# joekurina/Agilex-NTT

Measured on AMD Instinct MI355X. Metric: batched n=4096 forward NTTs/sec at 1/2/4/8 MI355X; %HBM roofline, higher is better.
Workload: dtype u64; 1 GPU; n=4096, 4-prime RNS (60-bit), batch=4096 polynomials per GPU, forward negacyclic NTT in place (BASELINE.json configs[2]); n=4096, primes=4, batch_per_gpu=4096, slabs_rotated=4, clock_ramp_steps_before_warmup=2240, parallelism=batch-sharded x1, no collective

## Files before the change

### agilex-ntt_amd/csrc/modarith.hpp

```cpp
#pragma once
#include <hip/hip_runtime.h>
#include <cstdint>

#include "q60c_class.hpp"

namespace agx {

typedef ulonglong2 twpair;

__device__ __forceinline__ uint64_t mul_shoup_lazy(uint64_t y, uint64_t w, uint64_t wp, uint64_t q) {
    const uint64_t c = __umul64hi(y, wp);
    return w * y - c * q;
}

__device__ __forceinline__ uint64_t csub(uint64_t v, uint64_t m) { return v >= m ? v - m : v; }

__device__ __forceinline__ uint64_t reduce_4q(uint64_t v, uint64_t q, uint64_t q2) {
    return csub(csub(v, q2), q);
}

__device__ __forceinline__ void ct_butterfly(uint64_t& x, uint64_t& y, uint64_t w, uint64_t wp,
                                             uint64_t q, uint64_t q2) {
    const uint64_t tx = csub(x, q2);
    const uint64_t qv = mul_shoup_lazy(y, w, wp, q);
    x = tx + qv;
    y = tx + q2 - qv;
}

__device__ __forceinline__ void gs_butterfly(uint64_t& x, uint64_t& y, uint64_t w, uint64_t wp,
                                             uint64_t q, uint64_t q2) {
    const uint64_t s = csub(x + y, q2);
    const uint64_t d = x + q2 - y;
    x = s;
    y = mul_shoup_lazy(d, w, wp, q);
}

struct barrett128 {
    uint64_t q;
    uint64_t mu_hi, mu_lo;
};

__device__ __forceinline__ uint64_t mul_mod_barrett(uint64_t a, uint64_t b, const barrett128& k) {
    const uint64_t lo = a * b, hi = __umul64hi(a, b);
    const uint64_t est = hi * k.mu_hi + __umul64hi(hi, k.mu_lo) + __umul64hi(lo, k.mu_hi);
    uint64_t r = lo - est * k.q;
    r = csub(r, k.q << 1);
    return csub(r, k.q);
}


__device__ __forceinline__ uint64_t reduce_u64(uint64_t v, const barrett128& k) {
    return csub(v - __umul64hi(v, k.mu_hi) * k.q, k.q);
}

__device__ __forceinline__ uint64_t rescale_lift(uint64_t t, uint64_t h, uint64_t hq, uint64_t q_last, const barrett128& k) {
    const uint64_t a = reduce_u64(csub(t + h, q_last), k);
    return a - hq + (a < hq ? k.q : 0);
}
template <bool LAZY>
__device__ __forceinline__ uint64_t rescale_finish(uint64_t x, uint64_t z, uint64_t w, uint64_t wp, uint64_t q) {
    const uint64_t d = x + (LAZY ? q << 2 : q) - z;
    return csub(mul_shoup_lazy(d, w, wp, q), q);
}

__device__ __forceinline__ uint64_t basis_scale(uint64_t x, uint64_t w, uint64_t wp, uint64_t qi) {
    return csub(mul_shoup_lazy(x, w, wp, qi), qi);
}
__device__ __forceinline__ uint64_t basis_accumulate(uint64_t acc, uint64_t y, uint64_t c, uint64_t cp, uint64_t q, uint64_t q2) {
    return csub(acc + mul_shoup_lazy(y, c, cp, q), q2);
}


__device__ __forceinline__ uint64_t mad64(uint32_t a, uint32_t b, uint64_t c) { return (uint64_t)a * b + c; }
__device__ __forceinline__ uint64_t mul64(uint32_t a, uint32_t b) { return (uint64_t)a * b; }

template <int TAG>
__device__ __forceinline__ uint32_t opaque_one() {
    uint32_t one;
    if constexpr (TAG == 0) asm("s_mov_b32 %0, 1" : "=s"(one));
    else asm("s_movk_i32 %0, 0x1" : "=s"(one));
    return one;
}
__device__ __forceinline__ uint64_t add64_32(uint64_t c, uint32_t a, uint32_t one) { return (uint64_t)a * one + c; }

__device__ __forceinline__ uint64_t opaque_sgpr64(uint64_t v) {
    asm("" : "+s"(v));
    return v;
}

__device__ __forceinline__ uint64_t keep64(uint64_t v) {
    asm("" : "+v"(v));
    return v;
}

struct bf_consts {
    uint64_t q;
    uint64_t nq;
    uint64_t m;
    uint64_t nm;
    uint32_t one_a, one_b;
    float est_inv;
    uint32_t c, c8;
    uint32_t c2, p29;
    uint64_t mfold;
};

__device__ __forceinline__ uint64_t csub_sign(uint64_t x, const bf_consts& k) {
    const uint64_t d = x + k.nm;
    const uint32_t neg = (uint32_t)((int32_t)(uint32_t)(d >> 32) >> 31);
    typedef uint32_t u32x2 __attribute__((ext_vector_type(2)));
    u32x2 add;
    add.x = neg & (uint32_t)k.m;
    add.y = neg & (uint32_t)(k.m >> 32);
    return d + __builtin_bit_cast(uint64_t, add);
}

template <int VAR = 0>
__device__ __forceinline__ uint64_t fold_product(uint64_t tx, uint64_t y, uint64_t w, uint64_t c, const bf_consts& k) {
    const uint32_t y0 = (uint32_t)y, y1 = (uint32_t)(y >> 32), w0 = (uint32_t)w, w1 = (uint32_t)(w >> 32);
    const uint32_t c0 = (uint32_t)c, c1 = (uint32_t)(c >> 32), nq0 = (uint32_t)k.nq, nq1 = (uint32_t)(k.nq >> 32);
    uint64_t acc = mad64(w0, y0, tx);
    acc = mad64(nq0, c0, acc);
    if constexpr (VAR == 1) {
        const uint32_t z32 = w0 * y1 + w1 * y0 + nq1 * c0 + nq0 * c1;
        typedef uint32_t u32x2v __attribute__((ext_vector_type(2)));
        u32x2v av = __builtin_bit_cast(u32x2v, acc);
        av.y += z32;
        return __builtin_bit_cast(uint64_t, av);
    }
    uint64_t z = mul64(w0, y1);
    z = mad64(w1, y0, z);
    z = mad64(nq1, c0, z);
    z = keep64(mad64(nq0, c1, z));
    typedef uint32_t u32x2 __attribute__((ext_vector_type(2)));
    u32x2 a = __builtin_bit_cast(u32x2, acc);
    a.y += (uint32_t)z;
    return __builtin_bit_cast(uint64_t, a);
}

__device__ __forceinline__ void ct_butterfly_exact(uint64_t& x, uint64_t& y, uint64_t w, uint64_t wp, const bf_consts& k) {
    const uint32_t y0 = (uint32_t)y, y1 = (uint32_t)(y >> 32), p0 = (uint32_t)wp, p1 = (uint32_t)(wp >> 32);
    const uint64_t tx = csub(x, k.m);
    const uint32_t t = __umulhi(y0, p0);
    const uint64_t m1 = add64_32(mul64(p1, y0), t, k.one_a);
    const uint64_t m2 = add64_32(mul64(p0, y1), (uint32_t)m1, k.one_b);
    uint64_t c = add64_32(mul64(p1, y1), (uint32_t)(m1 >> 32), k.one_a);
    c = add64_32(c, (uint32_t)(m2 >> 32), k.one_b);
    const uint64_t xn = fold_product(tx, y, w, c, k);
    y = (tx << 1) + k.m - xn;
    x = xn;
}

__device__ __forceinline__ uint64_t csub_select(uint64_t x, const bf_consts& k) {
    const uint64_t d = x + k.nm;
    return (int64_t)d < 0 ? x : d;
}

template <bool SEL = false>
__device__ __forceinline__ void ct_butterfly_fast(uint64_t& x, uint64_t& y, uint64_t w, uint64_t wp, const bf_consts& k) {
    const uint32_t y0 = (uint32_t)y, y1 = (uint32_t)(y >> 32), p0 = (uint32_t)wp, p1 = (uint32_t)(wp >> 32);
    const uint64_t tx = SEL ? csub_select(x, k) : csub_sign(x, k);
    uint64_t c = mad64(p1, y1, (uint64_t)__umulhi(y0, p1));
    c = add64_32(c, __umulhi(y1, p0), k.one_b);
    const uint64_t xn = fold_product(tx, y, w, c, k);
    y = (tx << 1) + k.m - xn;
    x = xn;
}

__device__ __forceinline__ uint64_t csub_sign_c(uint64_t x, uint64_t m, uint64_t nm) {
    const uint64_t d = x + nm;
    const uint32_t neg = (uint32_t)((int32_t)(uint32_t)(d >> 32) >> 31);
    typedef uint32_t u32x2 __attribute__((ext_vector_type(2)));
    u32x2 add;
    add.x = neg & (uint32_t)m;
    add.y = neg & (uint32_t)(m >> 32);
    return d + __builtin_bit_cast(uint64_t, add);
}

struct final_consts {
    uint64_t q2, nq2, q1, nq1;
    uint64_t q8, nq8;
};

template <bool FAST, bool SEL = false>
__device__ __forceinline__ uint64_t reduce_final(uint64_t v, const bf_consts& k, const final_consts& f, bool lazy_out = false) {
    if constexpr (FAST && SEL) {
        const uint64_t d4 = v + k.nm;
        v = (int64_t)d4 < 0 ? v : d4;
        if (lazy_out) return v;
        const uint64_t d2 = v + f.nq2;
        v = (int64_t)d2 < 0 ? v : d2;
        const uint64_t d1 = v + f.nq1;
        return (int64_t)d1 < 0 ? v : d1;
    } else if constexpr (FAST) {
        v = csub_sign(v, k);
        if (lazy_out) return v;
        v = csub_sign_c(v, f.q2, f.nq2);
        return csub_sign_c(v, f.q1, f.nq1);
    } else {
        if (lazy_out) return v;
        v = csub(v, k.q << 1);
        return csub(v, k.q);
    }
}

struct lazy16_schedule {
    static constexpr int bound_in(int s) {
        int b = 4;
        for (int i = 0; i < s; ++i) b = next(b);
        return b;
    }
    static constexpr bool subtracts(int s) { return bound_in(s) + 4 > 16; }
    static constexpr int next(int b) { return (b + 4 > 16 ? (b - 8 > 8 ? b - 8 : 8) : b) + 4; }
};

struct lazy16_tailfree {
    static constexpr bool subtracts(int s, int total) { return s >= 2 && (((s ^ total) & 1) == 0); }
    static constexpr int bound_in(int s, int total) {
        int b = 4;
        for (int i = 0; i < s; ++i) {
            if (subtracts(i, total)) b = b - 8 > 8 ? b - 8 : 8;
            b += 4;
        }
        return b;
    }
    static constexpr bool valid(int total) {
        for (int s = 0; s < total; ++s) {
            const int in = bound_in(s, total);
            if (in > 16) return false;
            if (!subtracts(s, total) && in + 4 > 16) return false;
        }
        return total >= 3 && !subtracts(total - 1, total);
    }
};

__device__ __forceinline__ uint64_t csub_select_c(uint64_t x, uint64_t nm) {
    const uint64_t d = x + nm;
    return (int64_t)d < 0 ? x : d;
}

template <bool SEL, bool DO_CSUB, bool LAST = false, int VAR = 0>
__device__ __forceinline__ void ct_butterfly_lazy16(uint64_t& x, uint64_t& y, uint64_t w, uint64_t wp, const bf_consts& k,
                                                    const final_consts& f) {
    const uint32_t y0 = (uint32_t)y, y1 = (uint32_t)(y >> 32), p0 = (uint32_t)wp, p1 = (uint32_t)(wp >> 32);
    uint64_t tx = x;
    if constexpr (DO_CSUB || LAST) {
        if constexpr (SEL) tx = csub_select_c(tx, f.nq8);
        else tx = csub_sign_c(tx, f.q8, f.nq8);
    }
    if constexpr (LAST) {
        if constexpr (SEL) tx = csub_select_c(tx, k.nm);
        else tx = csub_sign(tx, k);
    }
    uint64_t c = mad64(p1, y1, (uint64_t)__umulhi(y0, p1));
    c = add64_32(c, __umulhi(y1, p0), k.one_b);
    const uint64_t xn = fold_product<VAR>(tx, y, w, c, k);
    y = (tx << 1) + k.m - xn;
    x = xn;
}

template <bool SEL>
__device__ __forceinline__ uint64_t reduce_final_lazy16(uint64_t v, const bf_consts& k, const final_consts& f, bool lazy_out) {
    if constexpr (SEL) {
        v = csub_select_c(v, k.nm);
        if (lazy_out) return v;
        v = csub_select_c(v, f.nq2);
        return csub_select_c(v, f.nq1);
    } else {
        v = csub_sign(v, k);
        if (lazy_out) return v;
        v = csub_sign_c(v, f.q2, f.nq2);
        return csub_sign_c(v, f.q1, f.nq1);
    }
}

template <bool SEL, int USE_EST = -1>
__device__ __forceinline__ uint64_t reduce_final_est(uint64_t v, const bf_consts& k, const final_consts& f, bool lazy_out) {
    static_assert(SEL, "select-based conditional subtract only");
    if (USE_EST == 1 || (USE_EST == -1 && k.est_inv != 0.0f)) {
        const uint32_t kq = (uint32_t)((float)(uint32_t)(v >> 32) * k.est_inv);
        typedef uint32_t u32x2 __attribute__((ext_vector_type(2)));
        u32x2 r = __builtin_bit_cast(u32x2, mad64(kq, (uint32_t)k.nq, v));
        r.y += kq * (uint32_t)(k.nq >> 32);
        const uint64_t r64 = __builtin_bit_cast(uint64_t, r);
        return lazy_out ? r64 : csub_select_c(r64, f.nq1);
    }
    v = csub_select_c(v, f.nq8);
    v = csub_select_c(v, k.nm);
    if (lazy_out) return v;
    v = csub_select_c(v, f.nq2);
    return csub_select_c(v, f.nq1);
}

struct q60c_tailfree {
    struct bound {
        int b, e;
    };
    static constexpr bound bound_in(int s, int total) {
        bound v{4, 0};
        for (int i = 0; i < s; ++i) {
            if (lazy16_tailfree::subtracts(i, total)) {
                v.b = v.b - 8 > 8 ? v.b - 8 : 8;
                v.e = v.e > 1 ? v.e : 1;
            }
            v.b += 4;
        }
        return v;
    }
    static constexpr bool valid(int total) {
        for (int s = 0; s <= total; ++s) {
            const bound v = bound_in(s, total);
            if (v.b > 16 || v.e > 1) return false;
        }
        return lazy16_tailfree::valid(total);
    }
};

__device__ __forceinline__ uint64_t csub_8q_q60c(uint64_t x, const bf_consts& k) {
    typedef uint32_t u32x2 __attribute__((ext_vector_type(2)));
    u32x2 v = __builtin_bit_cast(u32x2, x);
    uint32_t s = v.y >> 31;
    asm("" : "+v"(s));
    v.y &= 0x7fffffffu;
    return mad64(s, k.c8, __builtin_bit_cast(uint64_t, v));
}

template <bool DO_CSUB>
__device__ __forceinline__ void ct_butterfly_q60c(uint64_t& x, uint64_t& y, uint64_t w, uint64_t wp, const bf_consts& k) {
    const uint32_t y0 = (uint32_t)y, y1 = (uint32_t)(y >> 32), p0 = (uint32_t)wp, p1 = (uint32_t)(wp >> 32);
    const uint64_t tx = DO_CSUB ? csub_8q_q60c(x, k) : x;
    uint64_t c = mad64(p1, y1, (uint64_t)__umulhi(y0, p1));
    c = add64_32(c, __umulhi(y1, p0), k.one_b);
    const uint64_t xn = fold_product(tx, y, w, c, k);
    y = (tx << 1) + k.m - xn;
    x = xn;
}

template <bool PIN = false>
__device__ __forceinline__ uint64_t reduce_top4_q60c(uint64_t x, const bf_consts& k) {
    typedef uint32_t u32x2 __attribute__((ext_vector_type(2)));
    u32x2 r = __builtin_bit_cast(u32x2, x);
    uint32_t kq = r.y >> 28;
    if constexpr (PIN) asm("" : "+v"(kq));
    r.y &= 0x0fffffffu;
    return mad64(kq, k.c, __builtin_bit_cast(uint64_t, r));
}
__device__ __forceinline__ uint64_t reduce_final_q60c(uint64_t v, const bf_consts& k, const final_consts& f, bool lazy_out) {
    const uint64_t t = reduce_top4_q60c(v, k);
    return lazy_out ? t : csub_select_c(t, f.nq1);
}

struct q60c_fold_bounds {
    typedef unsigned __int128 u128;
    static constexpr u128 two64 = (u128)1 << 64, w32 = 0xffffffffull;
    static constexpr u128 c_max = (1ull << 28) - 1, q_min = (1ull << 60) - (uint64_t)c_max, q_max = (1ull << 60) - 1;
    static constexpr u128 wh_max = (uint64_t)q_max >> 29, wl_max = (1ull << 29) - 1;
    static constexpr u128 hi_max = 2 * w32 * wh_max;
    static constexpr u128 lo_max = 2 * w32 * wl_max;
    static constexpr u128 Q_max = lo_max + w32 * ((u128)1 << 29) + w32 * 2 * c_max;
    static constexpr u128 tx_max = ((u128)1 << 63) + 8 * c_max - 1, tx_max_c1 = ((u128)1 << 63) + 8 - 1;
    static_assert(wh_max < ((u128)1 << 31), "the high half of a twiddle fits 31 bits");
    static_assert(hi_max < two64, "hi fits 64 bits");
    static_assert(tx_max + Q_max < two64, "x' = tx + Q does not wrap (every partial sum of the chain is below this one)");
    static_assert(Q_max <= 8 * q_min, "y' = tx + 8q - Q is not negative");
    static_assert(tx_max + 8 * q_min < two64 && tx_max_c1 + 8 * q_max < two64, "y' <= tx + 8q = 2^64 - 1 for every c");
};

__device__ __forceinline__ uint32_t opaque_two29() {
    uint32_t v;
    asm("s_mov_b32 %0, 0x20000000" : "=s"(v));
    return v;
}

struct q60c_skip_schedule {
    static constexpr bool reduces(int s) { return (s & 1) == 0; }
    static constexpr bool valid(int total) {
        for (int s = 1; s < total; ++s)
            if (!reduces(s) && !reduces(s - 1)) return false;
        return total >= 1 && reduces(0);
    }
};
struct q60c_skip_bounds {
    typedef unsigned __int128 u128;
    using F = q60c_fold_bounds;
    static constexpr u128 two64 = F::two64, w32 = F::w32;
    static constexpr u128 c_max = kQ60cSkipMaxC, q_min = (1ull << 60) - (uint64_t)c_max;
    static constexpr u128 Q_max = F::lo_max + w32 * ((u128)1 << 29) + w32 * 2 * c_max;
    static constexpr u128 r_max = ((u128)1 << 60) - 1 + 15 * c_max;
    static constexpr u128 out1_max = r_max + 7 * q_min;
    static_assert(c_max < ((u128)1 << 28), "a subclass of the moduli of q60c_fold_bounds: hi and the halves of a twiddle are bounded there");
    static_assert(15 * c_max < ((u128)1 << 32), "the fold's product fits a word");
    static_assert(Q_max <= 7 * q_min, "y' = tx + 7q - Q is not negative, on either kind of stage");
    static_assert(out1_max == ((u128)1 << 63) + 8 * c_max - 1, "8q + 16c - 1");
    static_assert(r_max + Q_max < two64, "reducing stage: x' does not wrap (every partial sum of the chain is below this one)");
    static_assert(out1_max + Q_max < two64, "the stage behind it: x' does not wrap (every partial sum of the chain is below this one)");
    static_assert(out1_max + 7 * q_min < two64, "... and y' <= tx + 7q = 15 2^60 + c - 1 (grows with c) stays below 2^64");
};

template <int FORM>
__device__ __forceinline__ void ct_butterfly_q60c_fold(uint64_t& x, uint64_t& y, uint64_t w, uint64_t wC, const bf_consts& k) {
    static_assert(FORM >= 0 && FORM <= 3, "no such form");
    const uint32_t y0 = (uint32_t)y, y1 = (uint32_t)(y >> 32);
    const uint32_t wl = (uint32_t)w, wh = (uint32_t)(w >> 32), wCl = (uint32_t)wC, wCh = (uint32_t)(wC >> 32);
    const uint64_t tx = FORM == 1 ? csub_8q_q60c(x, k) : FORM == 2 ? reduce_top4_q60c<true>(x, k) : x;
    const uint64_t hi = mad64(y1, wCh, mul64(y0, wh));
    uint64_t xn = keep64(mad64(y0, wl, tx));
    xn = mad64(y1, wCl, xn);
    xn = mad64((uint32_t)hi, k.p29, xn);
    xn = mad64((uint32_t)(hi >> 32), k.c2, xn);
    y = (tx << 1) + k.mfold - xn;
    x = xn;
}

template <bool FAST>
__device__ __forceinline__ uint64_t mul_shoup_form(uint64_t d, uint64_t w, uint64_t wp, const bf_consts& k) {
    const uint32_t d0 = (uint32_t)d, d1 = (uint32_t)(d >> 32), p0 = (uint32_t)wp, p1 = (uint32_t)(wp >> 32);
    uint64_t c;
    if constexpr (FAST) {
        c = mad64(p1, d1, (uint64_t)__umulhi(d0, p1));
        c = add64_32(c, __umulhi(d1, p0), k.one_b);
    } else {
        const uint32_t t = __umulhi(d0, p0);
        const uint64_t m1 = add64_32(mul64(p1, d0), t, k.one_a);
        const uint64_t m2 = add64_32(mul64(p0, d1), (uint32_t)m1, k.one_b);
        c = add64_32(mul64(p1, d1), (uint32_t)(m1 >> 32), k.one_a);
        c = add64_32(c, (uint32_t)(m2 >> 32), k.one_b);
    }
    return fold_product(0, d, w, c, k);
}

template <bool FAST, bool SEL = false>
__device__ __forceinline__ void gs_butterfly_form(uint64_t& x, uint64_t& y, uint64_t w, uint64_t wp, const bf_consts& k) {
    const uint64_t s = x + y;
    const uint64_t d = x + k.m - y;
    if constexpr (FAST) x = SEL ? csub_select(s, k) : csub_sign(s, k);
    else x = csub(s, k.m);
    y = mul_shoup_form<FAST>(d, w, wp, k);
}

template <bool FAST>
__device__ __forceinline__ void gs_last_form(uint64_t& x, uint64_t& y, uint64_t ninv, uint64_t ninv_p,
                                             uint64_t w1n, uint64_t w1n_p, const bf_consts& k) {
    const uint64_t s = x + y;
    const uint64_t d = x + k.m - y;
    x = mul_shoup_form<FAST>(s, ninv, ninv_p, k);
    y = mul_shoup_form<FAST>(d, w1n, w1n_p, k);
}

template <bool SEL>
__device__ __forceinline__ uint64_t csub_8q(uint64_t v, const final_consts& f) {
    return SEL ? csub_select_c(v, f.nq8) : csub_sign_c(v, f.q8, f.nq8);
}
constexpr int gs_bound(int B0, int s, int r) {
    if (s == 0) return B0;
    if ((r >> (s - 1)) & 1) return 4;
    const int b = gs_bound(B0, s - 1, r);
    return 2 * (b == 16 ? 8 : b);
}
template <int B, bool SEL>
__device__ __forceinline__ void gs_butterfly_lazy16(uint64_t& x, uint64_t& y, uint64_t w, uint64_t wp, const bf_consts& k, const final_consts& f) {
    static_assert(B == 4 || B == 8 || B == 16, "bounds are 4q, 8q or 16q");
    if constexpr (B == 16) {
        x = csub_8q<SEL>(x, f);
        y = csub_8q<SEL>(y, f);
    }
    const uint64_t s = x + y;
    const uint64_t d = x + (B == 4 ? k.m : f.q8) - y;
    y = mul_shoup_form<true>(d, w, wp, k);
    x = s;
}
template <int B, bool SEL>
__device__ __forceinline__ void gs_last_lazy16(uint64_t& x, uint64_t& y, uint64_t ninv, uint64_t ninv_p, uint64_t w1n, uint64_t w1n_p,
                                               const bf_consts& k, const final_consts& f) {
    if constexpr (B == 16) {
        x = csub_8q<SEL>(x, f);
        y = csub_8q<SEL>(y, f);
    }
    const uint64_t s = x + y;
    const uint64_t d = x + (B == 4 ? k.m : f.q8) - y;
    x = mul_shoup_form<true>(s, ninv, ninv_p, k);
    y = mul_shoup_form<true>(d, w1n, w1n_p, k);
}

template <bool FAST, bool SEL = false>
__device__ __forceinline__ uint64_t reduce_final_inv(uint64_t v, const bf_consts& k, const final_consts& f) {
    if constexpr (FAST && SEL) {
        v = csub_select_c(v, f.nq2);
        return csub_select_c(v, f.nq1);
    } else if constexpr (FAST) {
        v = csub_sign_c(v, f.q2, f.nq2);
        return csub_sign_c(v, f.q1, f.nq1);
    } else {
        return csub(v, k.q);
    }
}

}
```

### agilex-ntt_amd/csrc/rb_frame.hpp

```cpp
#pragma once
#include "rb_registry.hpp"
#include "modarith.hpp"

#include <algorithm>
#include <cstdlib>
#include <type_traits>
#include <utility>

#ifndef AGX_POLYMUL_MAXW
#define AGX_POLYMUL_MAXW 5
#endif
#ifndef AGX_TU
#error "define AGX_TU (a per-translation-unit namespace name) before including rb_frame.hpp / rb_kernels.hpp"
#endif

namespace agx {
namespace AGX_TU {



template <int B, int E, typename F>
__device__ __host__ __forceinline__ void static_for(F&& f) {
    if constexpr (B < E) {
        f(std::integral_constant<int, B>{});
        static_for<B + 1, E>(std::forward<F>(f));
    }
}

extern __shared__ __attribute__((aligned(16))) unsigned char agx_dyn_lds[];

template <int L, int R>
struct rb_geom {
    static constexpr int C = 1 << R;
    static constexpr int T = 1 << (L - R);
    static constexpr int NP = (L + R - 1) / R;
    static constexpr int rlo(int p) { return (L - R * (p + 1)) > 0 ? (L - R * (p + 1)) : 0; }
    static constexpr int hi(int p) { return L - 1 - R * p; }
    static constexpr int H(int p) { return 1 << (L - R - rlo(p)); }
    static constexpr int table_off(int p) { return p == 0 ? 0 : table_off(p - 1) + C * H(p - 1); }
    static constexpr int table_pairs = table_off(NP);
};

template <int L, int R>
struct rb2_geom : rb_geom<L, R> {
    using G = rb_geom<L, R>;
    static constexpr uint32_t elem(int p, uint32_t tid, uint32_t r) {
        const int rlo = G::rlo(p);
        return (tid & ((1u << rlo) - 1u)) | (r << rlo) | ((tid >> rlo) << (rlo + R));
    }
    static constexpr uint32_t owner(int p, uint32_t e) {
        const int rlo = G::rlo(p);
        return (e & ((1u << rlo) - 1u)) | ((e >> (rlo + R)) << rlo);
    }
    static constexpr bool exchange_is_wave_local(int p) {
        for (uint32_t tid = 0; tid < (uint32_t)G::T; ++tid)
            for (uint32_t r = 0; r < (uint32_t)G::C; ++r)
                if ((owner(p + 1, elem(p, tid, r)) >> 6) != (tid >> 6)) return false;
        return true;
    }
    static constexpr bool uniform_pass(int p) { return G::rlo(p) >= 6 || G::H(p) == 1; }
    static constexpr bool last_pass_wave_contiguous() { return G::rlo(G::NP - 1) == 0 && G::T >= 64; }
};

__device__ __forceinline__ twpair load_uniform(const twpair* p) {
    typedef const uint64_t __attribute__((address_space(4))) * const_ptr;
    const_ptr c = (const_ptr)(uintptr_t)p;
    twpair r;
    r.x = c[0];
    r.y = c[1];
    return r;
}

__device__ __forceinline__ void wave_lds_sync() {
    __builtin_amdgcn_fence(__ATOMIC_RELEASE, "wavefront");
    __builtin_amdgcn_wave_barrier();
    __builtin_amdgcn_fence(__ATOMIC_ACQUIRE, "wavefront");
}

struct bf_regs {
    int r0, r1, o;
};
template <int rb>
constexpr bf_regs bf_pair(int b) {
    const int r0 = ((b >> rb) << (rb + 1)) | (b & ((1 << rb) - 1));
    return {r0, r0 | (1 << rb), b >> rb};
}

struct no_op {
    __device__ __forceinline__ void operator()() const {}
};
template <int C, class WR, class RD, class SYNC, class MID = no_op>
__device__ __forceinline__ void split_words_out(const uint64_t (&x)[C], uint32_t* w, uint32_t (&lo)[C], WR&& wr, RD&& rd, SYNC&& sync, MID&& mid = MID{}) {
    static_for<0, C>([&](auto r) { w[wr(r)] = (uint32_t)x[r]; });
    mid();
    sync();
    static_for<0, C>([&](auto r) { lo[r] = w[rd(r)]; });
    sync();
    static_for<0, C>([&](auto r) { w[wr(r)] = (uint32_t)(x[r] >> 32); });
    sync();
}

constexpr int kOptPad = 1;
constexpr int kOptSelect = 2;
constexpr int kOptLazy16 = 16;
constexpr int kOptTwAhead = 32;
constexpr int kOptTrace = 64;
constexpr int kOptPrio = 128;
constexpr int kOptPrioBarrier = 512;
constexpr int kOptScalarBase = 1024;
constexpr int kOptLazyInv = 2048;
constexpr int kOptTwAheadInv = 4096;
constexpr int kOptNtLoad = 131072, kOptNtStore = 262144;
constexpr int kOptEstReduce = 524288;
constexpr int kOptSplitWord = 1048576;
constexpr int kOptStreamTw = 1 << 25;
constexpr int kOptPinBf = 1 << 26;
constexpr int kOptQ60c = 1 << 27;
constexpr int kOptQ60cFold = 1 << 28;
constexpr int kOptQ60cSkip = 1 << 21;
constexpr int kOptStreamCh1 = 1 << 29;

#ifdef AGX_DIAG
__device__ uint64_t* g_trace_buf = nullptr;
__device__ uint64_t g_trace_waves = 0;
#endif

template <int L, int R, bool FAST, int OPT = 0>
struct rb2_frame {
    using G = rb2_geom<L, R>;
    static constexpr int C = G::C, T = G::T, NP = G::NP;
    static constexpr bool FAST_ARITH = FAST, SEL = (OPT & kOptSelect) != 0, LAZY16 = FAST && (OPT & kOptLazy16) != 0;
    static_assert((OPT & kOptPad) != 0, "every kernel uses the padded image");
    static constexpr bool TWA = (OPT & kOptTwAhead) != 0 && R >= 3;
    static constexpr bool TRACE = (OPT & kOptTrace) != 0;
    static constexpr bool PRIO = (OPT & kOptPrio) != 0;
    static constexpr bool PRIO_BARRIER = PRIO && (OPT & kOptPrioBarrier) != 0, SCALAR_BASE = (OPT & kOptScalarBase) != 0;
    static constexpr bool LAZY_INV = LAZY16 && (OPT & kOptLazyInv) != 0;
    static constexpr bool NT_LOAD = (OPT & kOptNtLoad) != 0, NT_STORE = (OPT & kOptNtStore) != 0;
    static constexpr bool TWA_INV = (OPT & kOptTwAheadInv) != 0 && R == 3;
    static constexpr bool EST = LAZY16 && SEL && (OPT & kOptEstReduce) != 0;
    static constexpr bool Q60C = EST && (OPT & kOptQ60c) != 0;
    static constexpr bool Q60C_FOLD = Q60C && (OPT & kOptQ60cFold) != 0;
    static_assert((OPT & kOptQ60cFold) == 0 || Q60C, "the two-twiddle butterfly is a form of the q = 2^60 - c kernels");
    static constexpr bool Q60C_SKIP = Q60C_FOLD && (OPT & kOptQ60cSkip) != 0;
    static_assert((OPT & kOptQ60cSkip) == 0 || Q60C_FOLD, "the reduction on every second stage is a form of the two-twiddle butterfly");
    static_assert(!Q60C_SKIP || q60c_skip_schedule::valid(L), "no unreduced stage may follow another, and stage 0 reduces");
    static constexpr bool SPLIT = (OPT & kOptSplitWord) != 0;
    static constexpr bool STREAM_TW = (OPT & kOptStreamTw) != 0, PIN_BF = (OPT & kOptPinBf) != 0, STREAM_CH1 = (OPT & kOptStreamCh1) != 0;
    static_assert(!EST || lazy16_tailfree::valid(L), "tail-free schedule must keep every stage within 16q");
    static_assert(!Q60C || q60c_tailfree::valid(L), "sign-bit subtracts must keep every stage within 16q + 8c");
    mutable uint64_t ts[12];
    uint64_t trace_wave = ~0ull;
    bool trace_wait_stores = true;
    template <int I>
    __device__ __forceinline__ void stamp(uint64_t& anchor) const {
        if constexpr (TRACE) {
            uint64_t t;
            asm volatile("s_memtime %0\n\ts_waitcnt lgkmcnt(0)" : "=s"(t), "+v"(anchor) : : "memory");
            ts[I] = t;
        }
    }
    __device__ __forceinline__ void trace_flush() const {
#ifndef AGX_DIAG
        static_assert(!TRACE, "kOptTrace kernels belong to the diagnostics library (AGX_DIAG): the product library has no trace buffer");
#else
        if constexpr (TRACE) {
            const uint64_t wave = ((uint64_t)blockIdx.y * gridDim.x + blockIdx.x) * (blockDim.x >> 6) + (threadIdx.x >> 6);
            if ((threadIdx.x & 63u) == 0 && g_trace_buf != nullptr && wave < g_trace_waves) {
                uint64_t* dst = g_trace_buf + wave * 16;
#pragma unroll
                for (int i = 0; i < 12; ++i) dst[i] = ts[i];
                dst[12] = __builtin_amdgcn_s_getreg((31 << 11) | 4);
                dst[13] = __builtin_amdgcn_s_getreg((31 << 11) | 20);
            }
        }
#endif
    }
    static constexpr bool lane_full_pass(int p) { return p >= 0 && p < NP && G::rlo(p) < 6 && G::hi(p) - G::rlo(p) + 1 == R; }
    static constexpr int PADS = SPLIT ? 5 : 4;
    static constexpr uint32_t slab_elems = (1u << L) + (L >= PADS ? (1u << (L >= PADS ? L - PADS : 0)) : 0u);
    static constexpr uint32_t image_bytes = slab_elems * (SPLIT ? 4u : 8u);
    static __device__ __forceinline__ constexpr uint32_t img(uint32_t e) { return e + (e >> PADS); }
    uint32_t tid;
    bool lazy_out = false;
    uint64_t* slab;
    bf_consts k;
    final_consts fc;

    __device__ __forceinline__ void init_consts(uint64_t q, uint64_t est = 0) {
        k.est_inv = __uint_as_float((uint32_t)est);
        k.q = q;
        k.nq = 0 - q;
        k.m = FAST ? (q << 2) : (q << 1);
        k.nm = opaque_sgpr64(0 - k.m);
        k.one_a = opaque_one<0>();
        k.one_b = opaque_one<1>();
        fc.q2 = q << 1;
        fc.nq2 = opaque_sgpr64(0 - fc.q2);
        fc.q1 = q;
        fc.nq1 = opaque_sgpr64(0 - fc.q1);
        fc.q8 = q << 3;
        fc.nq8 = opaque_sgpr64(0 - fc.q8);
        if constexpr (Q60C) {
            k.c = (uint32_t)(est >> 32);
            k.c8 = k.c << 3;
        }
        if constexpr (Q60C_FOLD) {
            k.c2 = k.c << 1;
            k.p29 = opaque_two29();
            if constexpr (Q60C_SKIP) k.mfold = opaque_sgpr64((q << 3) - q);
            else k.mfold = q << 3;
        }
    }

    template <int stage>
    __device__ __forceinline__ void butterfly(uint64_t& a, uint64_t& b, const twpair& w) const {
        if constexpr (Q60C_SKIP) ct_butterfly_q60c_fold<(q60c_skip_schedule::reduces(stage) ? 2 : 3)>(a, b, w.x, w.y, k);
        else if constexpr (Q60C_FOLD) ct_butterfly_q60c_fold<(stage >= 1 ? 1 : 0)>(a, b, w.x, w.y, k);
        else if constexpr (Q60C) ct_butterfly_q60c<lazy16_tailfree::subtracts(stage, L)>(a, b, w.x, w.y, k);
        else if constexpr (EST) ct_butterfly_lazy16<SEL, lazy16_tailfree::subtracts(stage, L), false>(a, b, w.x, w.y, k, fc);
        else if constexpr (LAZY16) ct_butterfly_lazy16<SEL, lazy16_schedule::subtracts(stage), stage == L - 1>(a, b, w.x, w.y, k, fc);
        else if constexpr (FAST) ct_butterfly_fast<SEL>(a, b, w.x, w.y, k);
        else ct_butterfly_exact(a, b, w.x, w.y, k);
    }

    template <int stage, int MODE>
    __device__ __forceinline__ void forward_step(uint64_t& a, uint64_t& b, const twpair& w) const {
        butterfly<stage>(a, b, w);
        if constexpr (stage == L - 1) {
            a = final_reduce<MODE>(a);
            b = final_reduce<MODE>(b);
        }
    }
    template <int gap, int BND, class TW>
    __device__ __forceinline__ void inverse_step(uint64_t& a, uint64_t& b, const prime_consts& pc, TW&& tw) const {
        if constexpr (gap == L - 1) {
            if constexpr (LAZY_INV) gs_last_lazy16<BND, SEL>(a, b, pc.n_inv, pc.n_inv_p, pc.w1n, pc.w1n_p, k, fc);
            else gs_last_form<FAST>(a, b, pc.n_inv, pc.n_inv_p, pc.w1n, pc.w1n_p, k);
            a = reduce_final_inv<FAST, SEL>(a, k, fc);
            b = reduce_final_inv<FAST, SEL>(b, k, fc);
        } else {
            const twpair w = tw();
            if constexpr (LAZY_INV) gs_butterfly_lazy16<BND, SEL>(a, b, w.x, w.y, k, fc);
            else gs_butterfly_form<FAST, SEL>(a, b, w.x, w.y, k);
        }
    }
    static constexpr int inv_b0(int p) { return p == NP - 1 ? 4 : 8; }
    template <int p>
    __device__ __forceinline__ void inverse_pass_cleanup(uint64_t (&x)[C]) const {
        if constexpr (LAZY_INV && p > 0) {
            static_for<0, C>([&](auto Rr) {
                constexpr int r = Rr;
                if constexpr (gs_bound(inv_b0(p), G::hi(p) - G::rlo(p) + 1, r) == 16) x[r] = csub_8q<SEL>(x[r], fc);
            });
        }
    }

    template <int MODE>
    __device__ __forceinline__ uint64_t final_reduce(uint64_t v) const {
        if constexpr (Q60C) return reduce_final_q60c(v, k, fc, MODE == 4 ? lazy_out : (MODE & 1) != 0);
        if constexpr (MODE == 4) {
            if constexpr (EST) return reduce_final_est<SEL>(v, k, fc, lazy_out);
            else if constexpr (LAZY16) return reduce_final_lazy16<SEL>(v, k, fc, lazy_out);
            else return reduce_final<FAST, SEL>(v, k, fc, lazy_out);
        }
        if constexpr (EST) return reduce_final_est<SEL, (MODE & 2) ? 1 : 0>(v, k, fc, (MODE & 1) != 0);
        else if constexpr (LAZY16) return reduce_final_lazy16<SEL>(v, k, fc, (MODE & 1) != 0);
        else return reduce_final<FAST, SEL>(v, k, fc, (MODE & 1) != 0);
    }
    template <class Body>
    __device__ __forceinline__ void with_final_mode(Body&& body) const {
        if constexpr (!STREAM_TW) {
            body(std::integral_constant<int, 4>{});
            return;
        }
        if (lazy_out) {
            if constexpr (EST && !Q60C) {
                if (k.est_inv != 0.0f) body(std::integral_constant<int, 3>{});
                else body(std::integral_constant<int, 1>{});
            } else body(std::integral_constant<int, 1>{});
        } else {
            if constexpr (EST && !Q60C) {
                if (k.est_inv != 0.0f) body(std::integral_constant<int, 2>{});
                else body(std::integral_constant<int, 0>{});
            } else body(std::integral_constant<int, 0>{});
        }
    }

    template <int p>
    __device__ __forceinline__ uint32_t sbase() const {
        constexpr int rlo = G::rlo(p);
        return img((tid & ((1u << rlo) - 1u)) | ((tid >> rlo) << (rlo + R)));
    }

    template <int p>
    struct tw_src {
        twpair tw[C];
        const twpair* col;
        uint32_t hstride;
    };
    template <int p>
    __device__ __forceinline__ void fetch(tw_src<p>& t, const twpair* tbl) const {
        constexpr int rlo = G::rlo(p), H = G::H(p);
        const uint32_t high = tid >> rlo;
        if constexpr (G::uniform_pass(p)) {
            const uint32_t hcol = (uint32_t)__builtin_amdgcn_readfirstlane((int)high);
            const twpair* ucol = tbl + G::table_off(p) + (size_t)hcol * C;
            if constexpr (STREAM_TW) {
                t.col = ucol;
            } else {
#pragma unroll
                for (int j = 1; j < C; ++j) t.tw[j] = load_uniform(ucol + j);
                t.col = nullptr;
            }
            t.hstride = 0;
        } else {
            t.col = tbl;
            t.hstride = (uint32_t)H;
        }
    }
    template <int p>
    __device__ __forceinline__ twpair lane_entry(const twpair* tbl, int j) const {
        constexpr int rlo = G::rlo(p), H = G::H(p);
        if constexpr (!STREAM_TW) {
            const twpair* col = tbl + G::table_off(p) + (tid >> rlo);
            return col[(size_t)j * (uint32_t)H];
        }
        const twpair* base = tbl + G::table_off(p) + (size_t)j * (uint32_t)H;
        return base[tid >> rlo];
    }
    template <int p>
    __device__ __forceinline__ twpair twiddle(const tw_src<p>& t, int j) const {
        if constexpr (G::uniform_pass(p)) return t.tw[j];
        else return lane_entry<p>(t.col, j);
    }

    template <int p>
    __device__ __forceinline__ void image_read(uint64_t (&x)[C]) const {
        const uint32_t sb = sbase<p>();
        static_for<0, C>([&](auto Rr) { constexpr int r = Rr; x[r] = slab[sb + img((uint32_t)r << G::rlo(p))]; });
    }
    template <int p>
    __device__ __forceinline__ void image_write(const uint64_t (&x)[C]) const {
        const uint32_t sb = sbase<p>();
        static_for<0, C>([&](auto Rr) { constexpr int r = Rr; slab[sb + img((uint32_t)r << G::rlo(p))] = x[r]; });
    }
    template <int p>
    __device__ __forceinline__ void exchange_sync() const {
        if constexpr (!G::exchange_is_wave_local(p)) __syncthreads();
        else wave_lds_sync();
    }

    template <int from, int to>
    __device__ __forceinline__ void split_exchange(uint64_t (&x)[C]) const {
        static_assert(to == from + 1 || to == from - 1, "neighbouring passes");
        uint32_t* w = reinterpret_cast<uint32_t*>(slab);
        const uint32_t sb = sbase<from>(), nb = sbase<to>();
        auto rd = [&](auto r) { return nb + img((uint32_t)r << G::rlo(to)); };
        uint32_t lo[C];
        split_words_out(x, w, lo, [&](auto r) { return sb + img((uint32_t)r << G::rlo(from)); }, rd, [&] { exchange_sync<(from < to ? from : to)>(); });
        static_for<0, C>([&](auto r) { x[r] = (uint64_t)lo[r] | ((uint64_t)w[rd(r)] << 32); });
    }

    static constexpr int CH = STREAM_CH1 ? 1 : R >= 5 ? 2 : 4;
    static constexpr int st_kk(int ns, int S, bool inv = false) { return inv ? R - 1 - S : R - ns + S; }
    static constexpr int st_chunks_in_stage(int ns, int S, bool inv = false) { return (1 << st_kk(ns, S, inv)) > CH ? (1 << st_kk(ns, S, inv)) / CH : 1; }
    static constexpr int st_total(int ns, bool inv = false) { int t = 0; for (int S = 0; S < ns; ++S) t += st_chunks_in_stage(ns, S, inv); return t; }
    static constexpr int st_stage(int ns, int q, bool inv = false) { int S = 0; while (q >= st_chunks_in_stage(ns, S, inv)) { q -= st_chunks_in_stage(ns, S, inv); ++S; } return S; }
    static constexpr int st_chunk(int ns, int q, bool inv = false) { int S = 0; while (q >= st_chunks_in_stage(ns, S, inv)) { q -= st_chunks_in_stage(ns, S, inv); ++S; } return q; }
    static constexpr int st_count(int ns, int S, bool inv = false) { return (1 << st_kk(ns, S, inv)) < CH ? (1 << st_kk(ns, S, inv)) : CH; }
    struct tw_chunk {
        twpair e[CH];
    };
    template <int p, int q, bool INV = false>
    __device__ __forceinline__ void stream_load(tw_chunk& c, const tw_src<p>& t) const {
        constexpr int ns = G::hi(p) - G::rlo(p) + 1, S = st_stage(ns, q, INV), cc = st_chunk(ns, q, INV), kk = st_kk(ns, S, INV);
        static_for<0, st_count(ns, S, INV)>([&](auto I) {
            constexpr int j = (1 << kk) + cc * CH + (int)I;
            if constexpr (G::uniform_pass(p)) c.e[I] = load_uniform(t.col + j);
            else c.e[I] = lane_entry<p>(t.col, j);
        });
    }
    template <int P0, int P1>
    __device__ __forceinline__ void forward_passes_streamed(uint64_t (&x)[C], const twpair* tbl) const {
        static_assert(P0 == 0 && P1 == NP, "whole transform");
        static_for<P0, P1>([&](auto P) {
            constexpr int p = P;
            constexpr int rlo = G::rlo(p), hi = G::hi(p), ns = hi - rlo + 1, NQ = st_total(ns);
            tw_src<p> t;
            fetch<p>(t, tbl);
            tw_chunk buf[2];
            stream_load<p, 0>(buf[0], t);
            if constexpr (p > 0 && !SPLIT) image_read<p>(x);
            static_for<0, NQ>([&](auto Qc) {
                constexpr int q = Qc;
                constexpr int S = st_stage(ns, q), cc = st_chunk(ns, q), cnt = st_count(ns, S);
                constexpr int rb = (hi - rlo) - S;
                constexpr bool last_stage = (rlo + rb) == 0;
                if constexpr (q + 1 < NQ) stream_load<p, q + 1>(buf[(q + 1) & 1], t);
                __builtin_amdgcn_sched_barrier(0);
                auto chunk_body = [&](auto M) {
                    static_for<(cc * CH) << rb, (cc * CH + cnt) << rb>([&](auto B) {
                        constexpr bf_regs bf = bf_pair<rb>(B);
                        constexpr int r0 = bf.r0, r1 = bf.r1;
                        if constexpr (PIN_BF) asm volatile("" : "+v"(x[r0]), "+v"(x[r1]));
                        forward_step<L - 1 - (rlo + rb), decltype(M)::value>(x[r0], x[r1], buf[q & 1].e[bf.o - cc * CH]);
                        if constexpr (PIN_BF) asm volatile("" : "+v"(x[r0]), "+v"(x[r1]));
                    });
                };
                if constexpr (last_stage) with_final_mode(chunk_body);
                else chunk_body(std::integral_constant<int, 0>{});
                __builtin_amdgcn_sched_barrier(0);
            });
            if constexpr (p < NP - 1) {
                if constexpr (SPLIT) split_exchange<p, p + 1>(x);
                else {
                    image_write<p>(x);
                    exchange_sync<p>();
                }
                if constexpr (PRIO_BARRIER && !G::exchange_is_wave_local(p)) __builtin_amdgcn_s_setprio(0);
            }
        });
    }

    template <int P0, int P1>
    __device__ __forceinline__ void forward_passes(uint64_t (&x)[C], const twpair* tbl) const {
        if constexpr (STREAM_TW) {
            forward_passes_streamed<P0, P1>(x, tbl);
            return;
        }
        twpair ahead[C / 2];
        static_for<P0, P1>([&](auto P) {
            constexpr int p = P;
            constexpr int rlo = G::rlo(p), hi = G::hi(p), ns = hi - rlo + 1;
            constexpr bool twa_here = TWA && lane_full_pass(p);
            constexpr bool twa_prev = TWA && p > P0 && lane_full_pass(p);
            constexpr bool twa_next = TWA && p + 1 < P1 && lane_full_pass(p + 1);
            tw_src<p> t;
            fetch<p>(t, tbl);
            twpair late[C / 2];
            if constexpr (twa_here) {
                if constexpr (!twa_prev) {
                    static_for<1, C / 2>([&](auto J) { constexpr int j = J; ahead[j] = lane_entry<p>(tbl, j); });
                }
                static_for<0, C / 2>([&](auto J) { constexpr int j = J; late[j] = lane_entry<p>(tbl, j + C / 2); });
            }
            if constexpr (p > 0 && !SPLIT) {
                if constexpr (p == P0) exchange_sync<p - 1>();
                image_read<p>(x);
                if constexpr (2 * p + 1 < 12) stamp<2 * p + 1>(x[C - 1]);
            }
            static_for<0, ns>([&](auto S) {
                constexpr int rb = (hi - rlo) - S;
                constexpr int kk = R - 1 - rb;
                constexpr bool last_stage = (rlo + rb) == 0;
                if constexpr (twa_next && S == (ns > 1 ? ns - 1 : 0)) {
                    constexpr int pn = p + 1;
                    static_for<1, C / 2>([&](auto J) { constexpr int j = J; ahead[j] = lane_entry<pn>(tbl, j); });
                }
                auto stage_body = [&](auto M) {
                    static_for<0, C / 2>([&](auto B) {
                        constexpr bf_regs bf = bf_pair<rb>(B);
                        constexpr int j = (1 << kk) + bf.o;
                        twpair w;
                        if constexpr (twa_here && j < C / 2) w = ahead[j];
                        else if constexpr (twa_here) w = late[j - C / 2];
                        else w = twiddle<p>(t, j);
                        forward_step<L - 1 - (rlo + rb), decltype(M)::value>(x[bf.r0], x[bf.r1], w);
                    });
                };
                if constexpr (last_stage) with_final_mode(stage_body);
                else stage_body(std::integral_constant<int, 0>{});
            });
            if constexpr (2 * p + 2 < 12) stamp<2 * p + 2>(x[C - 1]);
            if constexpr (p < NP - 1) {
                if constexpr (SPLIT) {
                    static_assert(!SPLIT || (P0 == 0 && P1 == NP), "split-word exchanges run the whole transform in one call");
                    split_exchange<p, p + 1>(x);
                    if constexpr (PRIO_BARRIER && !G::exchange_is_wave_local(p)) __builtin_amdgcn_s_setprio(0);
                } else {
                image_write<p>(x);
                if constexpr (p < P1 - 1) {
                    exchange_sync<p>();
                    if constexpr (PRIO_BARRIER && !G::exchange_is_wave_local(p)) __builtin_amdgcn_s_setprio(0);
                }
                }
            }
        });
    }
    __device__ __forceinline__ void forward(uint64_t (&x)[C], const twpair* tbl) const {
        forward_passes<0, NP>(x, tbl);
    }

    __device__ __forceinline__ void inverse_streamed(uint64_t (&x)[C], const twpair* itbl, const prime_consts& pc) const {
        static_for<0, NP>([&](auto Qp) {
            constexpr int p = NP - 1 - Qp;
            constexpr int rlo = G::rlo(p), hi = G::hi(p), ns = hi - rlo + 1, NQ = st_total(ns, true);
            tw_src<p> t;
            fetch<p>(t, itbl);
            tw_chunk buf[2];
            stream_load<p, 0, true>(buf[0], t);
            if constexpr (p < NP - 1 && !SPLIT) image_read<p>(x);
            static_for<0, NQ>([&](auto Qc) {
                constexpr int q = Qc;
                constexpr int S = st_stage(ns, q, true), cc = st_chunk(ns, q, true), cnt = st_count(ns, S, true);
                constexpr int rb = S;
                if constexpr (q + 1 < NQ) stream_load<p, q + 1, true>(buf[(q + 1) & 1], t);
                __builtin_amdgcn_sched_barrier(0);
                static_for<(cc * CH) << rb, (cc * CH + cnt) << rb>([&](auto Bf) {
                    constexpr bf_regs bf = bf_pair<rb>(Bf);
                    constexpr int r0 = bf.r0, r1 = bf.r1;
                    if constexpr (PIN_BF) asm volatile("" : "+v"(x[r0]), "+v"(x[r1]));
                    inverse_step<rlo + rb, gs_bound(inv_b0(p), rb, r0)>(x[r0], x[r1], pc, [&] { return buf[q & 1].e[bf.o - cc * CH]; });
                    if constexpr (PIN_BF) asm volatile("" : "+v"(x[r0]), "+v"(x[r1]));
                });
                __builtin_amdgcn_sched_barrier(0);
            });
            inverse_pass_cleanup<p>(x);
            if constexpr (p > 0) {
                if constexpr (SPLIT) split_exchange<p, p - 1>(x);
                else {
                    image_write<p>(x);
                    exchange_sync<p - 1>();
                }
            }
        });
    }

    __device__ __forceinline__ void inverse(uint64_t (&x)[C], const twpair* itbl, const prime_consts& pc) const {
        if constexpr (STREAM_TW) {
            inverse_streamed(x, itbl, pc);
            return;
        }
        twpair first[4];
        static_for<0, NP>([&](auto Q) {
            constexpr int p = NP - 1 - Q;
            constexpr int rlo = G::rlo(p), hi = G::hi(p);
            constexpr bool twa_have = TWA_INV && p < NP - 1 && lane_full_pass(p) && lane_full_pass(p + 1);
            constexpr bool twa_next = TWA_INV && p > 0 && lane_full_pass(p) && lane_full_pass(p - 1);
            tw_src<p> t;
            fetch<p>(t, itbl);
            if constexpr (p < NP - 1) {
                image_read<p>(x);
                if constexpr (2 + 2 * Q < 12) stamp<2 + 2 * Q>(x[C - 1]);
            }
            static_for<0, hi - rlo + 1>([&](auto S) {
                constexpr int rb = S;
                constexpr int kk = R - 1 - rb;
                if constexpr (twa_next && S == hi - rlo) {
                    constexpr int pn = p - 1;
                    static_for<0, 4>([&](auto J) { constexpr int jj = J; first[jj] = lane_entry<pn>(itbl, jj + 4); });
                }
                static_for<0, C / 2>([&](auto Bf) {
                    constexpr bf_regs bf = bf_pair<rb>(Bf);
                    constexpr int j = (1 << kk) + bf.o;
                    inverse_step<rlo + rb, gs_bound(inv_b0(p), rb, bf.r0)>(x[bf.r0], x[bf.r1], pc, [&] {
                        if constexpr (twa_have && j >= 4) return first[j - 4];
                        else return twiddle<p>(t, j);
                    });
                });
            });
            if constexpr (3 + 2 * Q < 12) stamp<3 + 2 * Q>(x[C - 1]);
            inverse_pass_cleanup<p>(x);
            if constexpr (p > 0) {
                image_write<p>(x);
                exchange_sync<p - 1>();
            }
        });
    }

    __device__ __forceinline__ void load_pass0(uint64_t (&x)[C], const uint64_t* p, int64_t base) const {
#pragma unroll
        for (int r = 0; r < C; ++r) x[r] = NT_LOAD ? __builtin_nontemporal_load(&p[base + tid + (uint32_t)r * T]) : p[base + tid + (uint32_t)r * T];
    }
    __device__ __forceinline__ void store_pass0(const uint64_t (&x)[C], uint64_t* p, int64_t base, bool live = true) const {
        if (live) {
#pragma unroll
            for (int r = 0; r < C; ++r) {
                if constexpr (NT_STORE) __builtin_nontemporal_store(x[r], &p[base + tid + (uint32_t)r * T]);
                else p[base + tid + (uint32_t)r * T] = x[r];
            }
        }
    }

    __device__ __forceinline__ void store_last_layout(const uint64_t (&x)[C], uint64_t* __restrict__ out, int64_t base, bool live) const {
        static_assert(G::last_pass_wave_contiguous(), "store path assumes a wave-contiguous last pass");
        if constexpr (SPLIT) {
            uint32_t* w = reinterpret_cast<uint32_t*>(slab);
            const uint32_t own32 = img(tid << R);
            const uint32_t e0 = ((tid >> 6) << (6 + R)) + (tid & 63u), s0 = img(e0);
            uint32_t lo[C];
            split_words_out(x, w, lo, [&](auto r) { return own32 + img((uint32_t)r); }, [&](auto r) { return s0 + img(64u * (uint32_t)r); }, [] { wave_lds_sync(); });
            if (live) {
                static_for<0, C>([&](auto Rr) {
                    constexpr int r = Rr;
                    const uint64_t v = (uint64_t)lo[r] | ((uint64_t)w[s0 + img(64u * (uint32_t)r)] << 32);
                    if constexpr (NT_STORE) __builtin_nontemporal_store(v, &out[base + e0 + 64u * (uint32_t)r]);
                    else out[base + e0 + 64u * (uint32_t)r] = v;
                });
            }
            return;
        }
        const uint32_t own = img(tid << R);
        static_for<0, C>([&](auto Rr) { constexpr int r = Rr; slab[own + img((uint32_t)r)] = x[r]; });
        wave_lds_sync();
        if constexpr (TRACE) {
            const uint32_t e0 = ((tid >> 6) << (6 + R)) + (tid & 63u), s0 = img(e0);
            uint64_t y[C];
            static_for<0, C>([&](auto Rr) { constexpr int r = Rr; y[r] = slab[s0 + img(64u * (uint32_t)r)]; });
            stamp<9>(y[C - 1]);
            if (live) static_for<0, C>([&](auto Rr) { constexpr int r = Rr; out[base + e0 + 64u * (uint32_t)r] = y[r]; });
            stamp<10>(y[0]);
            asm volatile("s_waitcnt vmcnt(0)" ::: "memory");
            stamp<11>(y[0]);
            trace_flush();
            return;
        }
        if (live) {
            const uint32_t e0 = ((tid >> 6) << (6 + R)) + (tid & 63u), s0 = img(e0);
            static_for<0, C>([&](auto Rr) {
                constexpr int r = Rr;
                if constexpr (NT_STORE) __builtin_nontemporal_store(slab[s0 + img(64u * (uint32_t)r)], &out[base + e0 + 64u * (uint32_t)r]);
                else out[base + e0 + 64u * (uint32_t)r] = slab[s0 + img(64u * (uint32_t)r)];
            });
        }
    }
    __device__ __forceinline__ void load_last_issue(uint64_t (&x)[C], const uint64_t* __restrict__ in, int64_t base) const {
        const uint32_t e0 = ((tid >> 6) << (6 + R)) + (tid & 63u);
#pragma unroll
        for (int r = 0; r < C; ++r)
            x[r] = NT_LOAD ? __builtin_nontemporal_load(&in[base + e0 + 64u * (uint32_t)r]) : in[base + e0 + 64u * (uint32_t)r];
    }
    __device__ __forceinline__ void load_last_stage(uint64_t (&x)[C], const uint64_t* __restrict__ in2, const barrett128& bk, int64_t base) const {
        const uint32_t e0 = ((tid >> 6) << (6 + R)) + (tid & 63u), s0 = img(e0);
        if constexpr (SPLIT) {
            uint32_t* w = reinterpret_cast<uint32_t*>(slab);
            const uint32_t own32 = img(tid << R);
#pragma unroll
            for (int r = 0; r < C; ++r) {
                uint64_t v = x[r];
                if (in2) {
                    const uint64_t u = NT_LOAD ? __builtin_nontemporal_load(&in2[base + e0 + 64u * (uint32_t)r]) : in2[base + e0 + 64u * (uint32_t)r];
                    v = mul_mod_barrett(reduce_4q(v, k.q, k.q << 1), reduce_4q(u, k.q, k.q << 1), bk);
                }
                if constexpr (!FAST) v = csub(v, k.m);
                x[r] = v;
            }
            uint32_t lo[C];
            split_words_out(
                x, w, lo, [&](auto r) { return s0 + img(64u * (uint32_t)r); }, [&](auto r) { return own32 + img((uint32_t)r); }, [] { wave_lds_sync(); },
                [] { if constexpr (PRIO) __builtin_amdgcn_s_setprio(0); });
            static_for<0, C>([&](auto Rr) { constexpr int r = Rr; x[r] = (uint64_t)lo[r] | ((uint64_t)w[own32 + img((uint32_t)r)] << 32); });
            return;
        }
#pragma unroll
        for (int r = 0; r < C; ++r) {
            uint64_t v = x[r];
            if (in2) {
                const uint64_t u = NT_LOAD ? __builtin_nontemporal_load(&in2[base + e0 + 64u * (uint32_t)r]) : in2[base + e0 + 64u * (uint32_t)r];
                v = mul_mod_barrett(reduce_4q(v, k.q, k.q << 1), reduce_4q(u, k.q, k.q << 1), bk);
            }
            if constexpr (!FAST) v = csub(v, k.m);
            slab[s0 + img(64u * (uint32_t)r)] = v;
        }
        if constexpr (PRIO) __builtin_amdgcn_s_setprio(0);
        wave_lds_sync();
        const uint32_t own = img(tid << R);
#pragma unroll
        for (int r = 0; r < C; ++r) x[r] = slab[own + img((uint32_t)r)];
    }
};

}
}
```

### agilex-ntt_amd/csrc/reg_s4096.hip

```cpp
#define AGX_TU tu_s4096
#include "rb_kernels.hpp"
#include "rb_stream_opts.hpp"

namespace agx {
namespace AGX_TU {
const rb_entry kEntries[] = {
    make_entry_single_fwd<12, 5, kLazy | (kOptPrio << 1), 4>(159),
    make_entry_single_fwd_q60c_skip<12, 5, kLazy | ((kOptPrio | kOptQ60c | kOptQ60cFold) << 1), 4>(165),
#ifdef AGX_DIAG
    make_entry_single_fwd<12, 5, kLazy | ((kOptPrio | kOptQ60c | kOptQ60cFold) << 1), 4>(168),
    make_entry_single_fwd<12, 5, kLazy | ((kOptPrio | kOptQ60c) << 1), 4>(167),
    make_entry_single<12, 5, kLazy | (kOptPrio << 1), 4>(147),
    make_entry_single<12, 4, kLazy | (kOptStreamCh1 << 1), 8>(161),
#endif
};
}

rb_span rb_entries_s4096() { return rb_span{AGX_TU::kEntries, sizeof(AGX_TU::kEntries) / sizeof(AGX_TU::kEntries[0])}; }

}
```

Baseline: 72.66 million NTT/s.

## Defer final q60c subtract to a rare wave-uniform branch; scalar twiddle bases

In the streamed q = 2^60 - c forward kernel, the last stage now runs in the unreduced mode and a wave ballot flags any coefficient whose top word could reach q. The final conditional subtract over all registers then runs only when some lane is flagged. Static asserts prove the flag is conservative across the prime class. Separately, non-uniform twiddle loads use a scalar 64-bit base that advances per chunk, plus a per-lane 32-bit offset, in place of full per-lane pointers, which cuts VALU address arithmetic. Both are enabled on the production entry 165, with diagnostic variants added to isolate each. The ballot adds SALU work per butterfly in the last stage.

```diff
diff --git a/agilex-ntt_amd/csrc/modarith.hpp b/agilex-ntt_amd/csrc/modarith.hpp
--- a/agilex-ntt_amd/csrc/modarith.hpp
+++ b/agilex-ntt_amd/csrc/modarith.hpp
@@ -366,6 +366,18 @@
     static_assert(tx_max + 8 * q_min < two64 && tx_max_c1 + 8 * q_max < two64, "y' <= tx + 8q = 2^64 - 1 for every c");
 };
 
+constexpr uint32_t kQ60cTailHi = 0x0fffffffu;
+struct q60c_tail_bounds {
+    typedef unsigned __int128 u128;
+    using F = q60c_fold_bounds;
+    static constexpr u128 t_max = ((u128)1 << 60) - 1 + 15 * F::c_max;
+    static_assert(15 * F::c_max < ((u128)1 << 32), "k c fits a word: the fold cannot carry t past bit 61");
+    static_assert(t_max < ((u128)1 << 63), "the sign test of the cold block's csub_select_c is exact");
+    static_assert((F::q_min >> 32) >= kQ60cTailHi, "t >= q implies hi32(t) >= 0x0FFFFFFF, for every c of the class (q falls as c grows)");
+    static_assert((((u128)kQ60cTailHi << 32) - 1) < F::q_min, "a coefficient that is not flagged is below q");
+};
+__device__ __forceinline__ uint64_t q60c_tail_flag(uint64_t t) { return __builtin_amdgcn_ballot_w64((uint32_t)(t >> 32) >= kQ60cTailHi); }
+
 __device__ __forceinline__ uint32_t opaque_two29() {
     uint32_t v;
     asm("s_mov_b32 %0, 0x20000000" : "=s"(v));
diff --git a/agilex-ntt_amd/csrc/rb_frame.hpp b/agilex-ntt_amd/csrc/rb_frame.hpp
--- a/agilex-ntt_amd/csrc/rb_frame.hpp
+++ b/agilex-ntt_amd/csrc/rb_frame.hpp
@@ -118,6 +118,8 @@
 constexpr int kOptQ60c = 1 << 27;
 constexpr int kOptQ60cFold = 1 << 28;
 constexpr int kOptQ60cSkip = 1 << 21;
+constexpr int kOptQ60cRareSub = 1 << 22;
+constexpr int kOptTwScalarBase = 1 << 23;
 constexpr int kOptStreamCh1 = 1 << 29;
 
 #ifdef AGX_DIAG
@@ -147,6 +149,9 @@
     static_assert(!Q60C_SKIP || q60c_skip_schedule::valid(L), "no unreduced stage may follow another, and stage 0 reduces");
     static constexpr bool SPLIT = (OPT & kOptSplitWord) != 0;
     static constexpr bool STREAM_TW = (OPT & kOptStreamTw) != 0, PIN_BF = (OPT & kOptPinBf) != 0, STREAM_CH1 = (OPT & kOptStreamCh1) != 0;
+    static constexpr bool RARE_SUB = Q60C && STREAM_TW && (OPT & kOptQ60cRareSub) != 0, TW_SBASE = STREAM_TW && (OPT & kOptTwScalarBase) != 0;
+    static_assert((OPT & kOptQ60cRareSub) == 0 || RARE_SUB, "the rare last subtract is a form of the streamed q = 2^60 - c kernels");
+    static_assert((OPT & kOptTwScalarBase) == 0 || TW_SBASE, "scalar table bases are a form of the streamed kernels");
     static_assert(!EST || lazy16_tailfree::valid(L), "tail-free schedule must keep every stage within 16q");
     static_assert(!Q60C || q60c_tailfree::valid(L), "sign-bit subtracts must keep every stage within 16q + 8c");
     mutable uint64_t ts[12];
@@ -298,6 +303,8 @@
         twpair tw[C];
         const twpair* col;
         uint32_t hstride;
+        uint64_t sb;
+        uint32_t voff;
     };
     template <int p>
     __device__ __forceinline__ void fetch(tw_src<p>& t, const twpair* tbl) const {
@@ -317,6 +324,10 @@
         } else {
             t.col = tbl;
             t.hstride = (uint32_t)H;
+            if constexpr (TW_SBASE) {
+                t.sb = reinterpret_cast<uint64_t>(tbl + G::table_off(p));
+                t.voff = (tid >> rlo) * (uint32_t)sizeof(twpair);
+            }
         }
     }
     template <int p>
@@ -372,9 +383,26 @@
     struct tw_chunk {
         twpair e[CH];
     };
+    static constexpr int st_first(int ns, int q, bool inv = false) { return (1 << st_kk(ns, st_stage(ns, q, inv), inv)) + st_chunk(ns, q, inv) * CH; }
     template <int p, int q, bool INV = false>
-    __device__ __forceinline__ void stream_load(tw_chunk& c, const tw_src<p>& t) const {
+    __device__ __forceinline__ void stream_load(tw_chunk& c, tw_src<p>& t) const {
         constexpr int ns = G::hi(p) - G::rlo(p) + 1, S = st_stage(ns, q, INV), cc = st_chunk(ns, q, INV), kk = st_kk(ns, S, INV);
+        if constexpr (TW_SBASE && !G::uniform_pass(p)) {
+            constexpr int H = G::H(p), step = st_first(ns, q, INV) - (q == 0 ? 0 : st_first(ns, q - 1, INV));
+            t.sb = opaque_sgpr64(t.sb + (int64_t)step * H * (int64_t)sizeof(twpair));
+            typedef uint64_t u64x2 __attribute__((ext_vector_type(2)));
+            typedef const u64x2 __attribute__((address_space(1))) * global_ptr;
+            typedef const unsigned char __attribute__((address_space(1))) * global_bytes;
+            static_assert(sizeof(u64x2) == sizeof(twpair), "one 16-byte load per entry");
+            asm("" : "+v"(t.voff));
+            const global_bytes lane = (global_bytes)t.sb + t.voff;
+            static_for<0, st_count(ns, S, INV)>([&](auto I) {
+                const u64x2 e = *(global_ptr)(lane + (uint32_t)I * H * (uint32_t)sizeof(twpair));
+                c.e[I].x = e.x;
+                c.e[I].y = e.y;
+            });
+            return;
+        }
         static_for<0, st_count(ns, S, INV)>([&](auto I) {
             constexpr int j = (1 << kk) + cc * CH + (int)I;
             if constexpr (G::uniform_pass(p)) c.e[I] = load_uniform(t.col + j);
@@ -384,6 +412,7 @@
     template <int P0, int P1>
     __device__ __forceinline__ void forward_passes_streamed(uint64_t (&x)[C], const twpair* tbl) const {
         static_assert(P0 == 0 && P1 == NP, "whole transform");
+        uint64_t tail_mask = 0;
         static_for<P0, P1>([&](auto P) {
             constexpr int p = P;
             constexpr int rlo = G::rlo(p), hi = G::hi(p), ns = hi - rlo + 1, NQ = st_total(ns);
@@ -404,7 +433,10 @@
                         constexpr bf_regs bf = bf_pair<rb>(B);
                         constexpr int r0 = bf.r0, r1 = bf.r1;
                         if constexpr (PIN_BF) asm volatile("" : "+v"(x[r0]), "+v"(x[r1]));
-                        forward_step<L - 1 - (rlo + rb), decltype(M)::value>(x[r0], x[r1], buf[q & 1].e[bf.o - cc * CH]);
+                        if constexpr (RARE_SUB && last_stage && decltype(M)::value == 0) {
+                            forward_step<L - 1 - (rlo + rb), 1>(x[r0], x[r1], buf[q & 1].e[bf.o - cc * CH]);
+                            tail_mask |= q60c_tail_flag(x[r0]) | q60c_tail_flag(x[r1]);
+                        } else forward_step<L - 1 - (rlo + rb), decltype(M)::value>(x[r0], x[r1], buf[q & 1].e[bf.o - cc * CH]);
                         if constexpr (PIN_BF) asm volatile("" : "+v"(x[r0]), "+v"(x[r1]));
                     });
                 };
@@ -421,6 +453,9 @@
                 if constexpr (PRIO_BARRIER && !G::exchange_is_wave_local(p)) __builtin_amdgcn_s_setprio(0);
             }
         });
+        if constexpr (RARE_SUB) {
+            if (tail_mask != 0) static_for<0, C>([&](auto Rr) { constexpr int r = Rr; x[r] = csub_select_c(x[r], fc.nq1); });
+        }
     }
 
     template <int P0, int P1>
diff --git a/agilex-ntt_amd/csrc/reg_s4096.hip b/agilex-ntt_amd/csrc/reg_s4096.hip
--- a/agilex-ntt_amd/csrc/reg_s4096.hip
+++ b/agilex-ntt_amd/csrc/reg_s4096.hip
@@ -6,8 +6,11 @@
 namespace AGX_TU {
 const rb_entry kEntries[] = {
     make_entry_single_fwd<12, 5, kLazy | (kOptPrio << 1), 4>(159),
-    make_entry_single_fwd_q60c_skip<12, 5, kLazy | ((kOptPrio | kOptQ60c | kOptQ60cFold) << 1), 4>(165),
+    make_entry_single_fwd_q60c_skip<12, 5, kLazy | ((kOptPrio | kOptQ60c | kOptQ60cFold | kOptQ60cRareSub | kOptTwScalarBase) << 1), 4>(165),
 #ifdef AGX_DIAG
+    make_entry_single_fwd_q60c_skip<12, 5, kLazy | ((kOptPrio | kOptQ60c | kOptQ60cFold) << 1), 4>(169),
+    make_entry_single_fwd_q60c_skip<12, 5, kLazy | ((kOptPrio | kOptQ60c | kOptQ60cFold | kOptQ60cRareSub) << 1), 4>(170),
+    make_entry_single_fwd_q60c_skip<12, 5, kLazy | ((kOptPrio | kOptQ60c | kOptQ60cFold | kOptTwScalarBase) << 1), 4>(171),
     make_entry_single_fwd<12, 5, kLazy | ((kOptPrio | kOptQ60c | kOptQ60cFold) << 1), 4>(168),
     make_entry_single_fwd<12, 5, kLazy | ((kOptPrio | kOptQ60c) << 1), 4>(167),
     make_entry_single<12, 5, kLazy | (kOptPrio << 1), 4>(147),
```

Result: faster. 74.10 million NTT/s (median of 6 runs) (+2.0%).
